# nirschl-lab/stain2stain

Measured on AMD Instinct MI355X. Metric: paired 256x256 stain tiles/sec (full CFM optimisation step), higher is better.
Workload: dtype bf16

## Files before the change

### include/stain2stain_hip.h

```cpp
#ifndef STAIN2STAIN_HIP_H
#define STAIN2STAIN_HIP_H

#ifdef __cplusplus
extern "C" {
#endif

#define S2S_OK 0
#define S2S_ERR_SHAPE (-1)
#define S2S_ERR_ALIGN (-2)
#define S2S_ERR_DTYPE (-3)
#define S2S_ERR_LAUNCH (-4)
#define S2S_ERR_NULL (-5)

#define S2S_BF16 0
#define S2S_F32 1

int s2s_conv3x3_stat_blocks(int dtype, int B, int H, int W, int Cout);
int s2s_conv3x3_nhwc(int dtype, const void* x0, int ld0, int c0, const void* x1, int ld1, int c1,
                     const void* w_packed, const float* bias, void* y, int ldy, float* stat_part,
                     const float* ep_scale, const float* ep_shift, int relu, int B, int H, int W, int Cout,
                     void* stream);

int s2s_conv3x3_ksplit(int dtype, int B, int H, int W, int Cout, int cin);
int s2s_conv3x3_nhwc_k(int dtype, const void* x0, int ld0, int c0, const void* x1, int ld1, int c1,
                       const void* w_packed, const float* bias, void* y, int ldy, float* stat_part,
                       const float* ep_scale, const float* ep_shift, int relu, float* kwork, int B, int H, int W,
                       int Cout, void* stream);
int s2s_conv3x3_stat_rows(int dtype, int B, int H, int W, int Cout, int c0, int c1, int ld0, int ld1, int has_bias);
int s2s_conv3x3_staged(int dtype, int B, int H, int W, int Cout, int c0, int c1, int ld0, int ld1, int ldy, int stats);
int s2s_conv3x3_family(int dtype, int B, int H, int W, int Cout, int c0, int c1, int ld0, int ld1, int ldy, int has_bias,
                       int has_affine, int stats, int stat_rows, int kwork);
int s2s_conv3x3_nhwc_s(int dtype, const void* x0, int ld0, int c0, const void* x1, int ld1, int c1, const void* w_packed,
                       const float* bias, void* y, int ldy, float* stat_part, int stat_rows, const float* ep_scale,
                       const float* ep_shift, int relu, float* kwork, int B, int H, int W, int Cout, void* stream);
int s2s_debug_conv_clock(long* out_host, int n);

int s2s_conv3x3_wgrad_splits(int dtype, int B, int H, int W, int Cin, int Cout);
int s2s_conv3x3_wgrad_nhwc(int dtype, const void* dy, int lddy, int Cout, const void* x0, int ld0, int c0,
                           const void* x1, int ld1, int c1, float* part, float* grad_oihw, int accumulate,
                           int B, int H, int W, void* stream);
int s2s_conv3x3_wgrad_phase(int dtype, const void* dy, int lddy, int Cout, const void* x0, int ld0, int c0,
                            const void* x1, int ld1, int c1, float* part, float* grad_oihw, int accumulate,
                            int B, int H, int W, int phases, void* stream);

int s2s_stem_stat_blocks(int B, int H, int W);
int s2s_stem_conv3x3_fwd(int dtype, const float* x_nchw, const float* w_oihw, const float* bias, void* y, int ldy,
                         float* stat_part, int B, int H, int W, int Cin, int Cout, void* stream);
int s2s_stem_wgrad_blocks(int B, int H, int W);
int s2s_stem_conv3x3_wgrad(int dtype, const void* dy, int lddy, const float* x_nchw, float* part, float* dw_oihw,
                           float* dbias, int accumulate, int B, int H, int W, int Cin, int Cout, void* stream);
int s2s_head_conv1x1_fwd(int dtype, const void* x, int ldx, const float* w, const float* bias, float* y_nchw, int B,
                         int H, int W, int C, int Cout, void* stream);
int s2s_head_wgrad_blocks(int B, int H, int W);
int s2s_head_conv1x1_bwd(int dtype, const float* dy_nchw, const void* x, int ldx, const float* w, void* dx, int lddx,
                         float* part, float* dw, float* dbias, int accumulate, int B, int H, int W, int C, int Cout,
                         void* stream);

int s2s_head_loss_blocks(int B, int H, int W);
int s2s_head_loss_fused(int dtype, const void* x, int ldx, const float* w, const float* bias, const float* u_nchw,
                        float* v_nchw, void* dx, int lddx, float grad_scale, float* part, double* lpart, float* dw,
                        float* dbias, float* loss, int accumulate, int B, int H, int W, int C, int Cout, void* stream);

int s2s_tail_blocks(int B, int H, int W);
int s2s_tail_fwd_loss(int dtype, const void* raw, int ldx, const float* scale, const float* shift, const float* mean,
                      const float* invstd, const float* w, const float* bias, const float* u_nchw, float* v_nchw,
                      float* g_nchw, float grad_scale, float* part, double* lpart, float* bnwork, float* dw,
                      float* dbias, float* loss, float* dgamma, float* dbeta, float* conv_dbias, int accumulate, int B,
                      int H, int W, int C, int Cout, void* stream);
int s2s_tail_bwd_apply(int dtype, const void* raw, int ldx, const float* g_nchw, const float* w, const float* scale,
                       const float* shift, const float* mean, const float* invstd, const float* gamma,
                       const float* bnwork, void* dx, int lddx, int B, int H, int W, int C, int Cout, void* stream);

int s2s_bn_finalize(const float* part, int nblk, int C, long count, const float* gamma, const float* beta,
                    float* running_mean, float* running_var, long* num_batches_tracked, float momentum, float eps,
                    float* mean, float* invstd, float* scale, float* shift, void* stream);
int s2s_bn_finalize_b(const float* part, int nblk, int C, long count, const float* gamma, const float* beta,
                      float* running_mean, float* running_var, long* num_batches_tracked, float momentum, float eps,
                      float* mean, float* invstd, float* scale, float* shift, const float* conv_bias, void* stream);
int s2s_bn_eval_prepare(int C, const float* gamma, const float* beta, const float* running_mean,
                        const float* running_var, float eps, float* scale, float* shift, void* stream);
int s2s_bn_relu_apply(int dtype, const void* x, int ldx, const float* scale, const float* shift, void* y, int ldy,
                      void* pool, int ldp, int B, int H, int W, int C, void* stream);
int s2s_maxpool2(int dtype, const void* x, int ldx, void* pool, int ldp, int B, int H, int W, int C, void* stream);
int s2s_bn_bwd_blocks(int B, int H, int W, int C);
int s2s_bn_relu_bwd(int dtype, const void* g1, int ldg1, const void* gp, int ldgp, const float* scale,
                    const float* shift, const void* x, int ldx, const float* mean, const float* invstd, const float* gamma, float* dgamma,
                    float* dbeta, float* dbias_conv, int accumulate, void* dx, int lddx, float* work, int B, int H,
                    int W, int C, void* stream);
int s2s_bn_partial_sums(const float* part, int nblk, int C, float* sums, void* stream);
int s2s_bn_relu_bwd_phase(int dtype, const void* g1, int ldg1, const void* gp, int ldgp, const float* scale,
                          const float* shift, const void* x, int ldx, const float* mean, const float* invstd,
                          const float* gamma, float* dgamma, float* dbeta, float* dbias_conv, int accumulate, void* dx,
                          int lddx, float* work, int B, int H, int W, int C, long count_total, int phases, void* stream);

int s2s_upsample2x_bilinear_ac_fwd(int dtype, const void* x, int ldx, const float* bias_nc, void* y, int ldy, int B,
                                   int Hin, int Win, int Hout, int Wout, int C, void* stream);
int s2s_upsample2x_bilinear_ac_bwd(int dtype, const void* dy, int lddy, void* dx, int lddx, int B, int Hin, int Win,
                                   int Hout, int Wout, int C, void* stream);
int s2s_pixel_sum(int dtype, const void* x, int ldx, float* out_nc, int B, int HW, int C, int accumulate,
                  void* stream);

int s2s_time_embedding(const float* t, float* out, int B, int dim, void* stream);
int s2s_linear_fwd(const float* x, const float* w, const float* bias, float* y, int B, int K, int N, void* stream);
int s2s_linear_bwd(const float* dy, const float* x, const float* w, float* dx, float* dw, float* db, int accumulate,
                   int B, int K, int N, void* stream);
int s2s_silu_fwd(const float* h, float* a, int n, void* stream);
int s2s_silu_bwd(const float* h, const float* da, float* dh, int n, void* stream);
int s2s_cfm_sample(const float* x0, const float* x1, const float* t, const float* eps, float sigma, float* xt,
                   float* ut, int B, long per_sample, void* stream);
int s2s_mse_loss(const float* v, const float* u, float* dv, float grad_scale, float* loss, double* work, long count,
                 void* stream);
int s2s_ode_error_norm(const float* e, const float* y0, const float* y1, float atol, float rtol, float* out,
                       double* work, long n, void* stream);
int s2s_axpy(float* x, const float* y, float a, long n, void* stream);
int s2s_dp_partials(long n);
int s2s_dp_init(int phase, const float* y, const float* k1, const float* fa, double* state, double* part, float* out,
                float* t_out, int* status, float atol, float rtol, int B, long n, void* stream);
int s2s_dp_stage(int i, const float* y, const float* k1, const float* k2, const float* k3, const float* k4,
                 const float* k5, const float* k6, const double* state, float* out, float* t_out, int B, long n,
                 void* stream);
int s2s_dp_error(const float* k1, const float* k2, const float* k3, const float* k4, const float* k5, const float* k6,
                 const float* k7, const float* y, const float* y_new, const double* state, double* part, float atol,
                 float rtol, int B, long n, void* stream);
int s2s_dp_control(double* state, const double* part, int* status, int max_steps, int B, long n, void* stream);
int s2s_dp_commit(float* y, const float* y_new, float* k1, const float* k7, const double* state, int B, long n,
                  void* stream);
int s2s_rk_stage(const float* x, const float* k1, const float* k2, const float* k3, float c1, float c2, float c3, int nk,
                 float* out, float* t_out, const float* table, const int* counter, int stages, int stage, int table_len,
                 int B, long n, void* stream);
int s2s_rk_combine(float* x, const float* k1, const float* k2, const float* k3, const float* k4, float c1, float c2,
                   float c3, float c4, int nk, int* counter, int B, long n, void* stream);
int s2s_fill_f32(float* x, float v, long n, void* stream);
int s2s_euler_tick(float* t, int n, const float* table, int* counter, void* stream);

int s2s_adam_step(float* p, const float* g, float* m, float* v, long n, int step, float lr, float beta1, float beta2,
                  float eps, float weight_decay, float grad_scale, void* stream);
int s2s_adam_step_dev(float* p, const float* g, float* m, float* v, long n, const float* hyper, void* stream);
long s2s_adam_multi_blocks(long n);
int s2s_adam_multi(const void* desc, int ntensors, long total, int step, float lr, float beta1, float beta2, float eps,
                   float weight_decay, float grad_scale, void* stream);
int s2s_adam_ema_step(float* p, const float* g, float* m, float* v, float* ema, long n, int step, float lr, float beta1,
                      float beta2, float eps, float weight_decay, float grad_scale, float ema_weight, void* stream);
int s2s_adam_ema_step_dev(float* p, const float* g, float* m, float* v, float* ema, long n, const float* hyper,
                          const float* ema_weight, void* stream);
long s2s_ema_multi_blocks(long n);
int s2s_ema_multi(const void* desc, int ntensors, long total, const float* weight, void* stream);
long s2s_pack_conv3x3_fwd_elems(int Cout, int Cin);
long s2s_pack_conv3x3_dgrad_elems(int Cout, int Cin);
int s2s_pack_conv3x3(int dtype, const float* w_oihw, void* w_fwd, void* w_dgrad, int Cout, int Cin, void* stream);
int s2s_pack_conv3x3_batched(int dtype, const void* desc, int nlayers, long total, void* stream);
int s2s_nchw_to_nhwc(int dtype, const float* x_nchw, void* y, int ldy, int B, int C, int H, int W, void* stream);
int s2s_nhwc_to_nchw(int dtype, const void* x, int ldx, float* y_nchw, int accumulate, int B, int C, int H, int W,
                     void* stream);

int s2s_paired_crop_flip_normalize(const void* src_u8, const void* tgt_u8, const int* params, float* out_src,
                                   float* out_tgt, int B, int Hs, int Ws, int S, void* stream);
int s2s_pil_resize_bilinear_normalize(const void* src_u8, void* tmp_u8, const int* bounds_h, const int* kk_h,
                                      int ksize_h, const int* bounds_v, const int* kk_v, int ksize_v, void* out_u8,
                                      float* out_f, int B, int Hs, int Ws, int Ho, int Wo, void* stream);

int s2s_region_gather(const void* img_u8, long pitch, int H, int W, int band_top, int band_h, const int* origins,
                      float* out, int B, int T, void* stream);
int s2s_region_blend(const float* tiles, int c0, const float* tiles1, int c1, const int* origins, int n, int T,
                     int overlap, float* acc, int band_rows, int H, int W, int r0, int r1, void* stream);
int s2s_region_finalize(float* acc, int band_rows, int W, int C, int r0, int r1, void* out_u8, long pitch_u8,
                        float* out_f, long pitch_f, int out_top, void* stream);

int s2s_region_tissue_count(const void* img_u8, long pitch, int H, int W, int band_top, int band_h, const int* origins,
                            int n, int T, int white, int black, int* counts, void* stream);
int s2s_region_skip_weight(const int* origins, int n, int T, int overlap, float* ws, int band_rows, int H, int W,
                           int r0, int r1, void* stream);
int s2s_region_finalize_mixed(float* acc, float* ws, int band_rows, int W, int C, int r0, int r1, const void* src_u8,
                              long src_pitch, int src_top, void* out_u8, long pitch_u8, float* out_f, long pitch_f,
                              int out_top, void* stream);

int s2s_seg_loss(const float* z, const float* g, float* dz, float* out, double* work, long n, float smooth,
                 float dice_weight, float grad_scale, void* stream);
int s2s_seg_loss_multiclass(const float* z, const long* target, float* dz, float* out, double* work, long B, long HW,
                            int C, int ignore_index, float smooth, float dice_weight, float grad_scale, void* stream);

int s2s_seg_eval_binary(const float* z, const float* g, float* out, long* counts, double* work, long n, float smooth,
                        float dice_weight, void* stream);
int s2s_seg_eval_multiclass(const float* z, const long* target, float* out, long* counts, double* work, long B,
                            long HW, int C, int ignore_index, float smooth, float dice_weight, void* stream);
int s2s_head_mse_eval_blocks(int B, int H, int W, int C);
int s2s_head_mse_eval(int dtype, const void* x, int ldx, const float* w, const float* bias, const float* u_nchw,
                      float* loss, double* lpart, int B, int H, int W, int C, int Cout, void* stream);

int s2s_image_quality_blocks(int H, int W, int win);
int s2s_image_quality_f32(const float* a, const float* b, int B, int C, int H, int W, int quantize, int win,
                          const float* taps, float k1, float k2, double* part, void* stream);
int s2s_image_quality_u8(const void* a, long pitch_a, long img_a, const void* b, long pitch_b, long img_b, int B,
                         int band_top, int band_h, int H, int W, int by0, int nby, int win, const float* taps, float k1,
                         float k2, double* part, void* stream);
int s2s_image_quality_finalize(const double* part, int B, int C, int H, int W, int win, float range, float* out,
                               void* stream);

int s2s_stain_quant_chunks(int cell_h, int cell_w);
int s2s_stain_quant_u8(const void* a, long pitch_a, long img_a, const void* b, long pitch_b, long img_b, int paired,
                       int B, int band_top, int band_h, int H, int W, int cell_h, int cell_w, int g0, int ng,
                       const float* od_table, const float* unmix, int white, int black, int stain, double* part,
                       void* stream);
int s2s_stain_quant_f32(const float* a, const float* b, int paired, int B, int H, int W, const float* od_table,
                        const float* unmix, int white, int black, int stain, double* part, void* stream);
int s2s_stain_quant_finalize(const double* part, long owners, int nchunk, int paired, long* counts, double* sums,
                             float* out, void* stream);
int s2s_stain_separate(const void* img, int is_f32, long pitch, long img_stride, int B, int H, int W,
                       const float* od_table, const float* unmix, float* out, void* stream);

long s2s_stain_moments_slots(int B, int H, int W);
int s2s_stain_moments_u8(const void* img, long pitch, long img_stride, int B, int band_top, int band_h, int H, int W,
                         const int* q_table, int u_beta, int black, long* part, void* stream);
int s2s_stain_moments_finalize(const long* part, long nslots, long* out, void* stream);
int s2s_stain_angle_hist_u8(const void* img, long pitch, long img_stride, int B, int band_top, int band_h, int H, int W,
                            const float* od_table, const float* plane, int u_beta, int black, int reset, long* hist,
                            void* stream);
int s2s_stain_conc_hist_u8(const void* img, long pitch, long img_stride, int B, int band_top, int band_h, int H, int W,
                           const float* od_table, const float* unmix, int u_beta, int black, int reset, long* hist,
                           void* stream);
int s2s_stain_normalize_u8(const void* img, long pitch, long img_stride, int B, int H, int W, const float* od_table,
                           const float* coef, void* out, long out_pitch, long out_img, int out_f32, void* stream);

int s2s_weighted_mse(const float* v, const float* u, const float* mask, float* dv, float* out, double* work, long B,
                     int C, long HW, float roi_lambda, float grad_scale, void* stream);
int s2s_charbonnier_roi(const float* pred, const float* truth, const float* mask, float* out, double* work, long B,
                        int C, long HW, float eps_charb, float eps_area, void* stream);
int s2s_class_embed_add(const float* temb, const float* table, const long* y, float* out, int B, int dim,
                        void* stream);
int s2s_class_embed_bwd(const float* dout, const long* y, float* dtable, int accumulate, int B, int dim,
                        int num_classes, void* stream);

int s2s_instnorm_blocks(int B, int H, int W, int C);
int s2s_instnorm_lrelu_fwd(int dtype, const void* x, int ldx, const float* gamma, const float* beta, void* y, int ldy,
                           float* work, float* stats, int B, int H, int W, int C, float eps, float slope,
                           void* stream);
int s2s_instnorm_lrelu_bwd(int dtype, const void* g, int ldg, const void* x, int ldx, const float* stats, void* dx,
                           int lddx, float* dgamma, float* dbeta, int accumulate, float* work, int B, int H, int W,
                           int C, float slope, void* stream);

int s2s_conv2x2_stat_blocks(int B, int H, int W, int Cout);
int s2s_conv2x2_nhwc(int dtype, const void* x, int ldx, int cin, const void* w_packed, const float* bias, void* y,
                     int ldy, float* stat_part, int B, int H, int W, int Cout, int pad, void* stream);
int s2s_space_to_depth_pad1(int dtype, const void* x, int ldx, void* xs, int ldxs, int inverse, int B, int H, int W,
                            int C, void* stream);
int s2s_channel_sum_blocks(long npix, int C);
int s2s_channel_sum(int dtype, const void* x, int ldx, float* work, float* out, long npix, int C, int accumulate,
                    void* stream);
int s2s_pack_conv4x4(const float* w_oihw, void* wf, void* wd, int Cout, int Cin, int stride, void* stream);
int s2s_conv4x4s1_nhwc(int dtype, const void* x, int ldx, int cin, const void* w_packed, const float* bias, void* y,
                       int ldy, float* stat_part, int B, int H, int W, int Cout, int pad, void* stream);
int s2s_conv4x4s1_wgrad_splits(int B, int H, int W, int Cin, int Cout);
// ... 72 lines not shown
```

### stain2stain_amd/csrc/resample.hip

```cpp
#include "common.h"
#include <stdlib.h>

namespace {

struct Axis {
  int i0, i1;
  float w0, w1;
};

__device__ __forceinline__ Axis ac_axis(int dst, int n_in, float scale) {
  Axis a;
  const float src = scale * (float)dst;
  a.i0 = (int)src;
  if (a.i0 > n_in - 1) a.i0 = n_in - 1;
  a.i1 = a.i0 + (a.i0 < n_in - 1 ? 1 : 0);
  a.w1 = src - (float)a.i0;
  a.w0 = 1.f - a.w1;
  return a;
}

__device__ __forceinline__ int rs_pcb(int C) {
  int p = 1;
  while (p < 32 && p * 8 < C) p <<= 1;
  return p;
// ... 13 lines not shown
  const int nrows = B * Hout;
  for (int row0 = blockIdx.x * band; row0 < nrows; row0 += gridDim.x * band)
  for (int row = row0; row < row0 + band && row < nrows; ++row) {
    const int n = row / Hout, oy = row - n * Hout;
    const int uy = oy - padT;
    const bool row_in = uy >= 0 && uy < Hu;
    const Axis ay = ac_axis(row_in ? uy : 0, Hin, sh);
    const T* const r0 = x + ((long)n * Hin + ay.i0) * Win * ldx;
    const T* const r1 = x + ((long)n * Hin + ay.i1) * Win * ldx;
    T* const yr = y + (long)row * Wout * ldy;
    for (int pb = 0; pb < cp; pb += PCB) {
      const int c8 = (pb + pc) * 8;
      if (pb + pc >= cp) continue;
      float bv[8];
#pragma unroll
      for (int k = 0; k < 8; ++k) bv[k] = BIAS ? bias[(long)n * C + c8 + k] : 0.f;
      for (int ox = slot; ox < Wout; ox += WL) {
        const int ux = ox - padL;
        f32x8 o;
        if (!row_in || ux < 0 || ux >= Wu) {
#pragma unroll
          for (int k = 0; k < 8; ++k) o.v[k] = 0.f;
        } else {
          const Axis ax = ac_axis(ux, Win, sw);
          const int o0 = ax.i0 * ldx + c8, o1 = ax.i1 * ldx + c8;
          const f32x8 v00 = load8(r0 + o0), v01 = load8(r0 + o1), v10 = load8(r1 + o0), v11 = load8(r1 + o1);
#pragma unroll
          for (int k = 0; k < 8; ++k) {
            const float b = bv[k];
            o.v[k] = ay.w0 * (ax.w0 * (v00.v[k] + b) + ax.w1 * (v01.v[k] + b)) +
                     ay.w1 * (ax.w0 * (v10.v[k] + b) + ax.w1 * (v11.v[k] + b));
          }
        }
        store8(yr + ox * ldy + c8, o);
      }
    }
  }
}

template <typename T>
__global__ void upsample2x_bwd_kernel(const T* __restrict__ dy, int lddy, T* __restrict__ dx, int lddx, int B,
                                      int Hin, int Win, int Hout, int Wout, int padT, int padL, int C) {
  const int cp = C >> 3;
  const int Hu = 2 * Hin, Wu = 2 * Win;
  const float sh = Hu > 1 ? (float)(Hin - 1) / (float)(Hu - 1) : 0.f;
  const float sw = Wu > 1 ? (float)(Win - 1) / (float)(Wu - 1) : 0.f;
  const int total = B * Hin * Win * cp;
  for (int i = blockIdx.x * blockDim.x + threadIdx.x; i < total; i += gridDim.x * blockDim.x) {
    const int t0 = i / cp, c8 = (i - t0 * cp) * 8;
    const int t1 = t0 / Win, ix = t0 - t1 * Win;
    const int n = t1 / Hin, iy = t1 - n * Hin;
    int y_lo, y_hi, x_lo, x_hi;
    if (Hin == 1) { y_lo = 0; y_hi = Hu - 1; }
    else {
      y_lo = (int)floorf((float)(iy - 1) / sh) - 1; y_hi = (int)ceilf((float)(iy + 1) / sh) + 1;
      if (y_lo < 0) y_lo = 0;
      if (y_hi > Hu - 1) y_hi = Hu - 1;
    }
    if (Win == 1) { x_lo = 0; x_hi = Wu - 1; }
    else {
      x_lo = (int)floorf((float)(ix - 1) / sw) - 1; x_hi = (int)ceilf((float)(ix + 1) / sw) + 1;
      if (x_lo < 0) x_lo = 0;
      if (x_hi > Wu - 1) x_hi = Wu - 1;
    }
    constexpr int NSLOT = 12;
    float wxs[NSLOT];
#pragma unroll
    for (int j = 0; j < NSLOT; ++j) {
      const int ux = x_lo + j;
      float wx = 0.f;
      if (ux <= x_hi) {
        const Axis ax = ac_axis(ux, Win, sw);
        if (ax.i0 == ix) wx += ax.w0;
        if (ax.i1 == ix) wx += ax.w1;
        const int ox = ux + padL;
        if (ox < 0 || ox >= Wout) wx = 0.f;
      }
      wxs[j] = wx;
    }
    f32x8 acc;
#pragma unroll
    for (int k = 0; k < 8; ++k) acc.v[k] = 0.f;
    for (int uy = y_lo; uy <= y_hi; ++uy) {
      const Axis ay = ac_axis(uy, Hin, sh);
      float wy = 0.f;
      if (ay.i0 == iy) wy += ay.w0;
      if (ay.i1 == iy) wy += ay.w1;
      const int oy = uy + padT;
      if (wy == 0.f || oy < 0 || oy >= Hout) continue;
      const T* const rowp = dy + (((long)n * Hout + oy) * Wout + x_lo + padL) * lddy + c8;
#pragma unroll
      for (int j = 0; j < NSLOT; ++j) {
        if (wxs[j] == 0.f) continue;
        const f32x8 g = load8(rowp + (long)j * lddy);
        const float w = wy * wxs[j];
#pragma unroll
        for (int k = 0; k < 8; ++k) acc.v[k] += w * g.v[k];
      }
    }
    store8(dx + (((long)n * Hin + iy) * Win + ix) * lddx + c8, acc);
  }
}

__device__ __forceinline__ float ac_weight_of(int dst, int n_in, float scale, int src_index) {
  const Axis a = ac_axis(dst, n_in, scale);
  return (a.i0 == src_index ? a.w0 : 0.f) + (a.i1 == src_index ? a.w1 : 0.f);
}

template <typename T>
__global__ void upsample2x_bwd_win_kernel(const T* __restrict__ dy, int lddy, T* __restrict__ dx, int lddx, int B,
                                          int Hin, int Win, int Hout, int Wout, int padT, int padL, int C) {
  const int cp = C >> 3;
  const int Hu = 2 * Hin, Wu = 2 * Win;
  const float sh = (float)(Hin - 1) / (float)(Hu - 1), sw = (float)(Win - 1) / (float)(Wu - 1);
  const int total = B * Hin * Win * cp;
  for (int i = blockIdx.x * blockDim.x + threadIdx.x; i < total; i += gridDim.x * blockDim.x) {
    const int t0 = i / cp, c8 = (i - t0 * cp) * 8;
    const int t1 = t0 / Win, ix = t0 - t1 * Win;
    const int n = t1 / Hin, iy = t1 - n * Hin;
    int uy0 = (int)floorf((float)(iy - 1) / sh) - 1, ux0 = (int)floorf((float)(ix - 1) / sw) - 1;
    if (uy0 < 0) uy0 = 0;
    if (ux0 < 0) ux0 = 0;
    for (int t = 0; t < 8 && uy0 < Hu - 1 && ac_weight_of(uy0, Hin, sh, iy) == 0.f; ++t) ++uy0;
    for (int t = 0; t < 8 && ux0 < Wu - 1 && ac_weight_of(ux0, Win, sw, ix) == 0.f; ++t) ++ux0;
    float wy[5], wx[5];
    int oyc[5], oxc[5];
#pragma unroll
    for (int j = 0; j < 5; ++j) {
      const int uy = uy0 + j, ux = ux0 + j;
      const int oy = uy + padT, ox = ux + padL;
      wy[j] = (uy <= Hu - 1 && oy >= 0 && oy < Hout) ? ac_weight_of(uy, Hin, sh, iy) : 0.f;
      wx[j] = (ux <= Wu - 1 && ox >= 0 && ox < Wout) ? ac_weight_of(ux, Win, sw, ix) : 0.f;
      oyc[j] = oy < 0 ? 0 : (oy > Hout - 1 ? Hout - 1 : oy);
      oxc[j] = ox < 0 ? 0 : (ox > Wout - 1 ? Wout - 1 : ox);
    }
    f32x8 acc;
#pragma unroll
    for (int k = 0; k < 8; ++k) acc.v[k] = 0.f;
#pragma unroll
    for (int j = 0; j < 5; ++j) {
      const T* const rowp = dy + ((long)n * Hout + oyc[j]) * Wout * lddy + c8;
#pragma unroll
      for (int m = 0; m < 5; ++m) {
        const f32x8 g = load8(rowp + (long)oxc[m] * lddy);
        const float w = wy[j] * wx[m];
#pragma unroll
        for (int k = 0; k < 8; ++k) acc.v[k] = fmaf(w, g.v[k], acc.v[k]);
      }
    }
    store8(dx + (((long)n * Hin + iy) * Win + ix) * lddx + c8, acc);
  }
}

template <typename T>
__global__ void pixel_sum_kernel(const T* __restrict__ x, int ldx, float* __restrict__ out, int HW, int C,
                                 int accumulate) {
  const int n = blockIdx.y;
  const int c = blockIdx.x * 64 + (threadIdx.x & 63);
  const int rg = threadIdx.x >> 6;
  float s = 0.f;
  if (c < C)
    for (int p = rg; p < HW; p += 4) s += to_f32(x[((long)n * HW + p) * ldx + c]);
  __shared__ float red[4][64];
  red[rg][threadIdx.x & 63] = s;
  __syncthreads();
  if (rg == 0 && c < C) {
    s = red[0][threadIdx.x] + red[1][threadIdx.x] + red[2][threadIdx.x] + red[3][threadIdx.x];
    out[(long)n * C + c] = accumulate ? out[(long)n * C + c] + s : s;
  }
}

inline int ew_grid(long total) {
  long b = (total + 255) / 256;
  if (b > 8192) b = 8192;
  if (b < 1) b = 1;
  return (int)b;
}

}

extern "C" int s2s_upsample2x_bilinear_ac_fwd(int dtype, const void* x, int ldx, const float* bias_nc, void* y,
                                              int ldy, int B, int Hin, int Win, int Hout, int Wout, int C,
                                              void* stream) {
  if (!x || !y) return S2S_ERR_NULL;
  if (B <= 0 || Hin <= 0 || Win <= 0 || C <= 0 || (C % 8) || (ldx % 8) || (ldy % 8)) return S2S_ERR_SHAPE;
  if (Hout < 2 * Hin || Wout < 2 * Win) return S2S_ERR_SHAPE;
  const int padT = (Hout - 2 * Hin) / 2, padL = (Wout - 2 * Win) / 2;
  if ((long)Win * ldx >= (1L << 31) || (long)Wout * ldy >= (1L << 31) || (long)B * Hout >= (1L << 31))
    return S2S_ERR_SHAPE;
  hipStream_t s = (hipStream_t)stream;
  const long rows = (long)B * Hout;
  static const int band_env = [] { const char* e = getenv("S2S_UP_BAND"); return e ? atoi(e) : 0; }();
  const int band = band_env > 0 ? band_env : (rows >= 4096 ? 4 : rows >= 2048 ? 2 : 1);
  const long nwg = (rows + band - 1) / band;
  const dim3 grid((unsigned)(nwg < 65535 * 4 ? nwg : 65535 * 4));
#define S2S_UP(TT, BB)                                                                                          \
  hipLaunchKernelGGL((upsample2x_fwd_kernel<TT, BB>), grid, dim3(256), 0, s, (const TT*)x, ldx, bias_nc, (TT*)y, \
                     ldy, B, Hin, Win, Hout, Wout, padT, padL, C, band)
  if (dtype == S2S_BF16) { if (bias_nc) S2S_UP(bf16_t, true); else S2S_UP(bf16_t, false); }
  else if (dtype == S2S_F32) { if (bias_nc) S2S_UP(float, true); else S2S_UP(float, false); }
  else return S2S_ERR_DTYPE;
#undef S2S_UP
  S2S_LAUNCH_CHECK();
  return S2S_OK;
}

extern "C" int s2s_upsample2x_bilinear_ac_bwd(int dtype, const void* dy, int lddy, void* dx, int lddx, int B, int Hin,
                                              int Win, int Hout, int Wout, int C, void* stream) {
  if (!dy || !dx) return S2S_ERR_NULL;
  if (B <= 0 || Hin <= 0 || Win <= 0 || C <= 0 || (C % 8) || (lddy % 8) || (lddx % 8)) return S2S_ERR_SHAPE;
  if (Hout < 2 * Hin || Wout < 2 * Win) return S2S_ERR_SHAPE;
  const int padT = (Hout - 2 * Hin) / 2, padL = (Wout - 2 * Win) / 2;
  const long total = (long)B * Hin * Win * (C / 8);
  if (total >= (1L << 31) - (1L << 22)) return S2S_ERR_SHAPE;
  hipStream_t s = (hipStream_t)stream;
  const dim3 grid(ew_grid(total));
  const bool win = Hin > 3 && Win > 3;
  if (dtype != S2S_BF16 && dtype != S2S_F32) return S2S_ERR_DTYPE;
#define S2S_UPB(KERN, TT)                                                                                            \
  hipLaunchKernelGGL(KERN<TT>, grid, dim3(256), 0, s, (const TT*)dy, lddy, (TT*)dx, lddx, B, Hin, Win, Hout, Wout,   \
                     padT, padL, C)
  if (dtype == S2S_BF16) { if (win) S2S_UPB(upsample2x_bwd_win_kernel, bf16_t); else S2S_UPB(upsample2x_bwd_kernel, bf16_t); }
  else { if (win) S2S_UPB(upsample2x_bwd_win_kernel, float); else S2S_UPB(upsample2x_bwd_kernel, float); }
#undef S2S_UPB
  S2S_LAUNCH_CHECK();
  return S2S_OK;
}

extern "C" int s2s_pixel_sum(int dtype, const void* x, int ldx, float* out_nc, int B, int HW, int C, int accumulate,
                             void* stream) {
  if (!x || !out_nc) return S2S_ERR_NULL;
  if (B <= 0 || HW <= 0 || C <= 0) return S2S_ERR_SHAPE;
  hipStream_t s = (hipStream_t)stream;
  dim3 grid(cdiv(C, 64), B);
  if (dtype == S2S_BF16)
    hipLaunchKernelGGL(pixel_sum_kernel<bf16_t>, grid, dim3(256), 0, s, (const bf16_t*)x, ldx, out_nc, HW, C, accumulate);
  else if (dtype == S2S_F32)
    hipLaunchKernelGGL(pixel_sum_kernel<float>, grid, dim3(256), 0, s, (const float*)x, ldx, out_nc, HW, C, accumulate);
  else return S2S_ERR_DTYPE;
  S2S_LAUNCH_CHECK();
  return S2S_OK;
}
```

### stain2stain_amd/ops.py

```python
from __future__ import annotations

import contextlib
import ctypes
import os
import sys
from typing import Optional, Tuple

import torch

from . import _native

BF16, F32 = 0, 1


def _dt(t: torch.Tensor) -> int:
    if t.dtype == torch.bfloat16:
        return BF16
    if t.dtype == torch.float32:
        return F32
    raise RuntimeError(f"stain2stain_amd: unsupported activation dtype {t.dtype}")


_raw_stream = getattr(torch._C, "_cuda_getCurrentRawStream", None)
_raw_device = getattr(torch._C, "_cuda_getDevice", None)
# ... 370 lines not shown


def tail_fusable(C: int, cout: int) -> bool:
    pcb = C // 8
    return C % 8 == 0 and 1 <= pcb <= 64 and pcb & (pcb - 1) == 0 and 1 <= cout <= 4


@_timed("tail_fwd_loss")
def tail_fwd_loss(raw: torch.Tensor, stats: torch.Tensor, w: torch.Tensor, bias: Optional[torch.Tensor],
                  u_nchw: torch.Tensor, dw: torch.Tensor, dbias: Optional[torch.Tensor], dgamma: torch.Tensor,
                  dbeta: torch.Tensor, dbias_conv: Optional[torch.Tensor], want_v: bool = False,
                  grad_scale: float = 1.0, accumulate: bool = False):
    B, H, W, C = raw.shape
    cout = w.shape[0]
    if not tail_fusable(C, cout):
        raise RuntimeError(f"stain2stain_amd: the fused tail does not take C = {C}, cout = {cout}")
    px, ldx = _nhwc(raw)
    dev = raw.device
    g = torch.empty((B, cout, H, W), dtype=torch.float32, device=dev)
    v = torch.empty((B, cout, H, W), dtype=torch.float32, device=dev) if want_v else None
    nb = _L().s2s_tail_blocks(B, H, W)
    part = torch.empty((nb, cout, C + 1), dtype=torch.float32, device=dev)
    lpart = torch.empty((nb,), dtype=torch.float64, device=dev)
    work = torch.empty((2 * C * _L().s2s_bn_bwd_blocks(B, H, W, C) + 2 * C,), dtype=torch.float32, device=dev)
    loss = torch.empty((), dtype=torch.float32, device=dev)
    rc = _L().s2s_tail_fwd_loss(_dt(raw), px, ldx, stats[2].data_ptr(), stats[3].data_ptr(), stats[0].data_ptr(),
                                stats[1].data_ptr(), _f32(w.reshape(cout, C)), _f32(bias), _f32(u_nchw), _f32(v),
                                _f32(g), float(grad_scale), _f32(part), lpart.data_ptr(), _f32(work),
                                _f32(dw.reshape(cout, C)), _f32(dbias), loss.data_ptr(), _f32(dgamma), _f32(dbeta),
                                _f32(dbias_conv), int(accumulate), B, H, W, C, cout, _stream())
    _native.check(rc, "tail_fwd_loss")
    return loss, g, v, work


@_timed("tail_bwd_apply")
def tail_bwd_apply(raw: torch.Tensor, stats: torch.Tensor, w: torch.Tensor, g: torch.Tensor, gamma: torch.Tensor,
                   work: torch.Tensor) -> torch.Tensor:
    B, H, W, C = raw.shape
    cout = w.shape[0]
    px, ldx = _nhwc(raw)
    if tuple(g.shape) != (B, cout, H, W) or work.numel() != 2 * C * _L().s2s_bn_bwd_blocks(B, H, W, C) + 2 * C:
        raise RuntimeError("stain2stain_amd: tail_bwd_apply operands do not belong to this tail_fwd_loss")
    dx = torch.empty((B, H, W, C), dtype=raw.dtype, device=raw.device)
    rc = _L().s2s_tail_bwd_apply(_dt(raw), px, ldx, _f32(g), _f32(w.reshape(cout, C)), stats[2].data_ptr(),
                                 stats[3].data_ptr(), stats[0].data_ptr(), stats[1].data_ptr(), _f32(gamma),
                                 _f32(work), dx.data_ptr(), C, B, H, W, C, cout, _stream())
    _native.check(rc, "tail_bwd_apply")
    return dx


@_timed("bn_finalize")
def bn_finalize(stat: torch.Tensor, count: int, gamma, beta, running_mean, running_var, num_batches,
                momentum: float = 0.1, eps: float = 1e-5, conv_bias: Optional[torch.Tensor] = None):
    _, C, nblk = stat.shape
    dev = stat.device
    out = torch.empty((4, C), dtype=torch.float32, device=dev)
    rc = _L().s2s_bn_finalize_b(_f32(stat), nblk, C, count, _f32(gamma), _f32(beta), _f32(running_mean),
                                _f32(running_var), 0 if num_batches is None else num_batches.data_ptr(), momentum, eps,
                                out[0].data_ptr(), out[1].data_ptr(), out[2].data_ptr(), out[3].data_ptr(),
                                _f32(conv_bias), _stream())
    _native.check(rc, "bn_finalize")
    return out


def bn_partial_sums(stat: torch.Tensor) -> torch.Tensor:
    _, C, nblk = stat.shape
    sums = torch.empty((2, C), dtype=torch.float32, device=stat.device)
    _native.check(_L().s2s_bn_partial_sums(_f32(stat), nblk, C, _f32(sums), _stream()), "bn_partial_sums")
    return sums


def bn_eval_prepare(gamma, beta, rmean, rvar, eps: float = 1e-5):
    C = gamma.numel()
    out = torch.empty((2, C), dtype=torch.float32, device=gamma.device)
    rc = _L().s2s_bn_eval_prepare(C, _f32(gamma), _f32(beta), _f32(rmean), _f32(rvar), eps, out[0].data_ptr(),
                                  out[1].data_ptr(), _stream())
    _native.check(rc, "bn_eval_prepare")
    return out


@_timed("bn_relu_apply")
def bn_relu_apply(x: torch.Tensor, scale: torch.Tensor, shift: torch.Tensor, out: Optional[torch.Tensor] = None,
                  pool: Optional[torch.Tensor] = None, want_pool: bool = False):
    B, H, W, C = x.shape
    px, ldx = _nhwc(x)
    if out is None:
        out = torch.empty((B, H, W, C), dtype=x.dtype, device=x.device)
    py, ldy = _nhwc(out)
    pp, ldp = 0, 8
    if want_pool and pool is None:
        pool = torch.empty((B, H // 2, W // 2, C), dtype=x.dtype, device=x.device)
    if pool is not None:
        pp, ldp = _nhwc(pool)
    rc = _L().s2s_bn_relu_apply(_dt(x), px, ldx, _f32(scale), _f32(shift), py, ldy, pp, ldp, B, H, W, C, _stream())
    _native.check(rc, "bn_relu_apply")
    return out, pool


@_timed("maxpool2")
def maxpool2(x: torch.Tensor) -> torch.Tensor:
    B, H, W, C = x.shape
    px, ldx = _nhwc(x)
    pool = torch.empty((B, H // 2, W // 2, C), dtype=x.dtype, device=x.device)
    rc = _L().s2s_maxpool2(_dt(x), px, ldx, pool.data_ptr(), C, B, H, W, C, _stream())
    _native.check(rc, "maxpool2")
    return pool


@_timed("bn_relu_bwd")
def bn_relu_bwd(g1: Optional[torch.Tensor], gp: Optional[torch.Tensor], x: torch.Tensor,
                stats: torch.Tensor, gamma: torch.Tensor, dgamma: torch.Tensor, dbeta: torch.Tensor,
                dbias_conv: Optional[torch.Tensor], accumulate: bool = False, exchange=None,
                count_total: Optional[int] = None) -> torch.Tensor:
    B, H, W, C = x.shape
    px, ldx = _nhwc(x)
    p1, ld1 = (0, 8) if g1 is None else _nhwc(g1)
    p2, ld2 = (0, 8) if gp is None else _nhwc(gp)
    dx = torch.empty((B, H, W, C), dtype=x.dtype, device=x.device)
    nb = _L().s2s_bn_bwd_blocks(B, H, W, C)
    work = torch.empty((4 * nb * C + 2 * C,), dtype=torch.float32, device=x.device)
    if exchange is not None:
        for phase in (1, 2):
            rc = _L().s2s_bn_relu_bwd_phase(_dt(x), p1, ld1, p2, ld2, stats[2].data_ptr(), stats[3].data_ptr(), px, ldx,
                                            stats[0].data_ptr(), stats[1].data_ptr(),
                                            _f32(gamma), _f32(dgamma), _f32(dbeta), _f32(dbias_conv), int(accumulate),
                                            dx.data_ptr(), C, _f32(work), B, H, W, C,
                                            int(count_total if count_total is not None else B * H * W), phase, _stream())
            _native.check(rc, "bn_relu_bwd")
            if phase == 1:
                exchange(work[4 * nb * C:])
        return dx
    rc = _L().s2s_bn_relu_bwd(_dt(x), p1, ld1, p2, ld2, stats[2].data_ptr(), stats[3].data_ptr(), px, ldx,
                              stats[0].data_ptr(), stats[1].data_ptr(),
                              _f32(gamma), _f32(dgamma), _f32(dbeta), _f32(dbias_conv), int(accumulate),
                              dx.data_ptr(), C, _f32(work), B, H, W, C, _stream())
    _native.check(rc, "bn_relu_bwd")
    return dx


@_timed("upsample2x_fwd")
def upsample2x_fwd(x: torch.Tensor, out: torch.Tensor, bias_nc: Optional[torch.Tensor] = None) -> None:
    B, Hin, Win, C = x.shape
    _, Hout, Wout, Co = out.shape
    if Co != C or out.dtype != x.dtype:
        raise RuntimeError("stain2stain_amd: upsample output slice mismatch")
    px, ldx = _nhwc(x)
    py, ldy = _nhwc(out)
    rc = _L().s2s_upsample2x_bilinear_ac_fwd(_dt(x), px, ldx, _f32(bias_nc), py, ldy, B, Hin, Win, Hout, Wout, C,
                                             _stream())
    _native.check(rc, "upsample2x_fwd")


@_timed("upsample2x_bwd")
def upsample2x_bwd(dy: torch.Tensor, hin: int, win: int) -> torch.Tensor:
    B, Hout, Wout, C = dy.shape
    pdy, lddy = _nhwc(dy)
    dx = torch.empty((B, hin, win, C), dtype=dy.dtype, device=dy.device)
    rc = _L().s2s_upsample2x_bilinear_ac_bwd(_dt(dy), pdy, lddy, dx.data_ptr(), C, B, hin, win, Hout, Wout, C,
                                             _stream())
    _native.check(rc, "upsample2x_bwd")
    return dx


def pixel_sum(x: torch.Tensor) -> torch.Tensor:
    B, H, W, C = x.shape
    px, ldx = _nhwc(x)
    out = torch.empty((B, C), dtype=torch.float32, device=x.device)
    rc = _L().s2s_pixel_sum(_dt(x), px, ldx, _f32(out), B, H * W, C, 0, _stream())
    _native.check(rc, "pixel_sum")
    return out


def time_embedding(t: torch.Tensor, dim: int) -> torch.Tensor:
    t = t.reshape(-1).to(torch.float32).contiguous()
    out = torch.empty((t.numel(), dim), dtype=torch.float32, device=t.device)
    _native.check(_L().s2s_time_embedding(_f32(t), _f32(out), t.numel(), dim, _stream()), "time_embedding")
    return out


def linear_fwd(x: torch.Tensor, w: torch.Tensor, b: Optional[torch.Tensor]) -> torch.Tensor:
    B, K = x.shape
    N = w.shape[0]
    y = torch.empty((B, N), dtype=torch.float32, device=x.device)
    _native.check(_L().s2s_linear_fwd(_f32(x), _f32(w), _f32(b), _f32(y), B, K, N, _stream()), "linear_fwd")
    return y


def linear_bwd(dy: torch.Tensor, x: torch.Tensor, w: torch.Tensor, dw: torch.Tensor, db: Optional[torch.Tensor],
               need_dx: bool = True, accumulate: bool = False) -> Optional[torch.Tensor]:
    B, K = x.shape
    N = w.shape[0]
    dx = torch.empty((B, K), dtype=torch.float32, device=x.device) if need_dx else None
    _native.check(_L().s2s_linear_bwd(_f32(dy), _f32(x), _f32(w), _f32(dx), _f32(dw), _f32(db), int(accumulate), B, K,
                                      N, _stream()), "linear_bwd")
    return dx


def silu_fwd(h: torch.Tensor) -> torch.Tensor:
    a = torch.empty_like(h)
    _native.check(_L().s2s_silu_fwd(_f32(h), _f32(a), h.numel(), _stream()), "silu_fwd")
    return a


def silu_bwd(h: torch.Tensor, da: torch.Tensor) -> torch.Tensor:
    dh = torch.empty_like(h)
    _native.check(_L().s2s_silu_bwd(_f32(h), _f32(da), _f32(dh), h.numel(), _stream()), "silu_bwd")
    return dh


@_timed("cfm_sample")
def cfm_sample(x0: torch.Tensor, x1: torch.Tensor, t: torch.Tensor, sigma: float = 0.0,
               eps: Optional[torch.Tensor] = None):
    xt = torch.empty_like(x0)
    ut = torch.empty_like(x0)
    B = x0.shape[0]
    _native.check(_L().s2s_cfm_sample(_f32(x0), _f32(x1), _f32(t), _f32(eps), float(sigma), _f32(xt), _f32(ut), B,
                                      x0.numel() // B, _stream()), "cfm_sample")
    return xt, ut


@_timed("mse_loss")
def mse_loss(v: torch.Tensor, u: torch.Tensor, want_grad: bool = True, grad_scale: float = 1.0):
    loss = torch.empty((), dtype=torch.float32, device=v.device)
    dv = torch.empty_like(v) if want_grad else None
    work = torch.empty((1024,), dtype=torch.float64, device=v.device)
    _native.check(_L().s2s_mse_loss(_f32(v), _f32(u), _f32(dv), float(grad_scale), loss.data_ptr(), work.data_ptr(),
                                    v.numel(), _stream()), "mse_loss")
    return loss, dv


def seg_loss(z: torch.Tensor, g: torch.Tensor, smooth: float = 1.0, dice_weight: float = 0.5, want_grad: bool = True,
             grad_scale: float = 1.0):
    z = z.contiguous()
    g = g.to(torch.float32).contiguous()
    out = torch.empty((3,), dtype=torch.float32, device=z.device)
    dz = torch.empty_like(z) if want_grad else None
    work = torch.empty((512 * 4 + 4,), dtype=torch.float64, device=z.device)
    _native.check(_L().s2s_seg_loss(_f32(z), _f32(g), _f32(dz), _f32(out), work.data_ptr(), z.numel(), float(smooth),
                                    float(dice_weight), float(grad_scale), _stream()), "seg_loss")
    return out, dz


def seg_loss_multiclass(z: torch.Tensor, target: torch.Tensor, ignore_index: int = -100, smooth: float = 1.0,
                        dice_weight: float = 0.5, want_grad: bool = True, grad_scale: float = 1.0,
                        validate: bool = True):
    if z.dim() != 4 or target.dim() != 3 or target.shape != (z.shape[0], z.shape[2], z.shape[3]):
        raise RuntimeError("stain2stain_amd: seg_loss_multiclass wants logits [B,C,H,W] and target [B,H,W]")
    B, C, H, W = z.shape
    z = z.contiguous()
    target = target.to(torch.int64).contiguous()
    if validate:
        lo, hi = int(target.min()), int(target.max())
        if lo < 0 or hi >= C:
            raise RuntimeError(f"stain2stain_amd: class index out of range [0, {C}) in segmentation target "
                               f"(min {lo}, max {hi})")
    out = torch.empty((3,), dtype=torch.float32, device=z.device)
    dz = torch.empty_like(z) if want_grad else None
    work = torch.empty((513 * 26,), dtype=torch.float64, device=z.device)
    _native.check(_L().s2s_seg_loss_multiclass(_f32(z), target.data_ptr(), _f32(dz), _f32(out), work.data_ptr(), B,
                                               H * W, C, int(ignore_index), float(smooth), float(dice_weight),
                                               float(grad_scale), _stream()), "seg_loss_multiclass")
    return out, dz


EV_BLOCKS = 512


def _gpu_f32_operand(t: torch.Tensor, what: str) -> torch.Tensor:
    if not t.is_cuda:
        raise RuntimeError(f"stain2stain_amd: {what} is not on the GPU (there is no CPU path)")
    if t.dtype != torch.float32:
        raise RuntimeError(f"stain2stain_amd: {what} must be float32, got {t.dtype}")
    return t.contiguous()


def _binary_mask(g: torch.Tensor) -> torch.Tensor:
    if g.dtype in (torch.bool, torch.uint8):
        return g.to(torch.float32).contiguous()
    if g.dtype != torch.float32:
        raise RuntimeError(f"stain2stain_amd: mask must be float32 (0/1), uint8 or bool, got {g.dtype}")
    return g.contiguous()


@_timed("seg_eval_binary")
def seg_eval_binary(z: torch.Tensor, g: torch.Tensor, smooth: float = 1.0, dice_weight: float = 0.5):
    if z.dim() != 4 or z.shape[1] != 1:
        raise RuntimeError(f"stain2stain_amd: seg_eval_binary wants logits [B,1,H,W], got {tuple(z.shape)}")
    if g.dim() == 3:
        g = g.unsqueeze(1)
    if tuple(g.shape) != tuple(z.shape):
        raise RuntimeError(f"stain2stain_amd: mask shape {tuple(g.shape)} does not match logits {tuple(z.shape)}")
    if g.device != z.device:
        raise RuntimeError("stain2stain_amd: logits and mask are on different devices")
    z, g = _gpu_f32_operand(z, "logits"), _binary_mask(g)
    out = torch.empty((5,), dtype=torch.float32, device=z.device)
    counts = torch.empty((4,), dtype=torch.int64, device=z.device)
    work = _workspace(z.device, 2 * EV_BLOCKS * 8, "seg_eval").view(torch.float64)
    _native.check(_L().s2s_seg_eval_binary(_f32(z), _f32(g), _f32(out), counts.data_ptr(), work.data_ptr(), z.numel(),
                                           float(smooth), float(dice_weight), _stream()), "seg_eval_binary")
    return out, counts


@_timed("seg_eval_multiclass")
def seg_eval_multiclass(z: torch.Tensor, target: torch.Tensor, ignore_index: int = -100, smooth: float = 1.0,
                        dice_weight: float = 0.5):
    if z.dim() != 4:
        raise RuntimeError(f"stain2stain_amd: seg_eval_multiclass wants logits [B,C,H,W], got {tuple(z.shape)}")
    B, C, H, W = z.shape
    if not 2 <= C <= 8:
        raise RuntimeError(f"stain2stain_amd: seg_eval_multiclass supports 2 <= C <= 8 classes, got {C}")
    if target.dim() == 4 and target.shape[1] == 1:
        target = target[:, 0]
    if tuple(target.shape) != (B, H, W):
        raise RuntimeError(f"stain2stain_amd: target shape {tuple(target.shape)} does not match logits {tuple(z.shape)}")
# ... 1093 lines not shown
```

Before: 2300.

## Add 2x2-quad upsample backward kernel and unroll pixel_sum loads

Adds a new bilinear upsample backward kernel in which each thread computes a 2x2 quad of input pixels from a shared 6x6 window of output gradients. Neighbouring outputs reuse the same loads instead of each pixel gathering its own 5x5 window. The kernel also uses an XCD-aware workgroup remap and sched barriers. Separately, pixel_sum is unrolled by 16 so more loads are in flight. A reference path and a family-query entry point are kept for testing, at the cost of extra code and higher register pressure.

```diff
diff --git a/include/stain2stain_hip.h b/include/stain2stain_hip.h
--- a/include/stain2stain_hip.h
+++ b/include/stain2stain_hip.h
@@ -97,6 +97,9 @@
                                    int Hin, int Win, int Hout, int Wout, int C, void* stream);
 int s2s_upsample2x_bilinear_ac_bwd(int dtype, const void* dy, int lddy, void* dx, int lddx, int B, int Hin, int Win,
                                    int Hout, int Wout, int C, void* stream);
+int s2s_upsample2x_bilinear_ac_bwd_ref(int dtype, const void* dy, int lddy, void* dx, int lddx, int B, int Hin,
+                                       int Win, int Hout, int Wout, int C, void* stream);
+int s2s_upsample2x_bwd_family(int lddy, int lddx, int B, int Hin, int Win, int Hout, int Wout, int C, int reference);
 int s2s_pixel_sum(int dtype, const void* x, int ldx, float* out_nc, int B, int HW, int C, int accumulate,
                   void* stream);
 
diff --git a/stain2stain_amd/csrc/resample.hip b/stain2stain_amd/csrc/resample.hip
--- a/stain2stain_amd/csrc/resample.hip
+++ b/stain2stain_amd/csrc/resample.hip
@@ -189,6 +189,137 @@
   }
 }
 
+template <typename T> struct Raw8;
+template <> struct Raw8<bf16_t> { bf16x8 a; };
+template <> struct Raw8<float> { f32x4 a, b; };
+__device__ __forceinline__ Raw8<bf16_t> load_raw8(const bf16_t* p) {
+  Raw8<bf16_t> r;
+  r.a = *reinterpret_cast<const bf16x8*>(p);
+  return r;
+}
+__device__ __forceinline__ Raw8<float> load_raw8(const float* p) {
+  Raw8<float> r;
+  r.a = *reinterpret_cast<const f32x4*>(p);
+  r.b = *reinterpret_cast<const f32x4*>(p + 4);
+  return r;
+}
+__device__ __forceinline__ f32x8 widen8(const Raw8<bf16_t>& r) {
+  f32x8 o;
+#pragma unroll
+  for (int i = 0; i < 8; ++i) o.v[i] = (float)r.a[i];
+  return o;
+}
+__device__ __forceinline__ f32x8 widen8(const Raw8<float>& r) {
+  f32x8 o;
+#pragma unroll
+  for (int i = 0; i < 4; ++i) { o.v[i] = r.a[i]; o.v[4 + i] = r.b[i]; }
+  return o;
+}
+
+__device__ __forceinline__ void pin8(f32x8& r) {
+#pragma unroll
+  for (int i = 0; i < 8; ++i) asm volatile("" : "+v"(r.v[i]));
+}
+
+template <typename T>
+__global__ __launch_bounds__(256, sizeof(T) == 2 ? 4 : 2) void upsample2x_bwd_quad_kernel(const T* __restrict__ dy, int lddy,
+                                                                  T* __restrict__ dx, int lddx, int B, int Hin,
+                                                                  int Win, int Hout, int Wout, int padT, int padL,
+                                                                  int C, int nwork) {
+  const int cp = C >> 3;
+  const int Hu = 2 * Hin, Wu = 2 * Win;
+  const float sh = (float)(Hin - 1) / (float)(Hu - 1), sw = (float)(Win - 1) / (float)(Wu - 1);
+  const int PCB = rs_pcb(C), WL = 256 / PCB;
+  const int pc = threadIdx.x & (PCB - 1), slot = threadIdx.x / PCB;
+  const int HP = (Hin + 1) >> 1, WP = (Win + 1) >> 1;
+  const int nwg = gridDim.x, q = nwg >> 3, r = nwg & 7, cls = blockIdx.x & 7;
+  const int wgid = (cls < r ? cls * (q + 1) : r * (q + 1) + (cls - r) * q) + (blockIdx.x >> 3);
+  const int chunk = wgid / nwork, work = wgid - chunk * nwork;
+  const int n = work / HP, iy0 = min(2 * (work - n * HP), Hin - 2);
+  const int piece = chunk * PCB + pc;
+  if (piece >= cp) return;
+  const int c8 = piece * 8;
+
+  float wyA[4], wyB[4];
+  const T* rowp[6];
+#pragma unroll
+  for (int j = 0; j < 6; ++j) {
+    const int uy = 2 * iy0 - 1 + j;
+    const bool in = uy >= 0 && uy <= Hu - 1;
+    if (j < 4) wyA[j] = in ? ac_weight_of(uy, Hin, sh, iy0) : 0.f;
+    if (j >= 2) wyB[j - 2] = in ? ac_weight_of(uy, Hin, sh, iy0 + 1) : 0.f;
+    int oy = uy + padT;
+    oy = oy < 0 ? 0 : (oy > Hout - 1 ? Hout - 1 : oy);
+    rowp[j] = dy + ((long)n * Hout + oy) * Wout * lddy;
+  }
+  T* const dr0 = dx + ((long)n * Hin + iy0) * Win * lddx + c8;
+  T* const dr1 = dr0 + (long)Win * lddx;
+
+#pragma unroll 1
+  for (int px = slot; px < WP; px += WL) {
+    const int ix0 = min(2 * px, Win - 2);
+    float wxA[4], wxB[4];
+    int off[6];
+#pragma unroll
+    for (int m = 0; m < 6; ++m) {
+      const int ux = 2 * ix0 - 1 + m;
+      const bool in = ux >= 0 && ux <= Wu - 1;
+      if (m < 4) wxA[m] = in ? ac_weight_of(ux, Win, sw, ix0) : 0.f;
+      if (m >= 2) wxB[m - 2] = in ? ac_weight_of(ux, Win, sw, ix0 + 1) : 0.f;
+      int ox = ux + padL;
+      ox = ox < 0 ? 0 : (ox > Wout - 1 ? Wout - 1 : ox);
+      off[m] = ox * lddy + c8;
+    }
+    f32x8 a00, a01, a10, a11;
+#pragma unroll
+    for (int k = 0; k < 8; ++k) a00.v[k] = a01.v[k] = a10.v[k] = a11.v[k] = 0.f;
+#pragma unroll
+    for (int j = 0; j < 6; ++j) {
+      Raw8<T> cur[6];
+#pragma unroll
+      for (int m = 0; m < 6; ++m) cur[m] = load_raw8(rowp[j] + off[m]);
+      f32x8 g[6];
+#pragma unroll
+      for (int m = 0; m < 6; ++m) g[m] = widen8(cur[m]);
+      if (j < 4) {
+#pragma unroll
+        for (int m = 0; m < 4; ++m) {
+          const float w = wyA[j] * wxA[m];
+#pragma unroll
+          for (int k = 0; k < 8; ++k) a00.v[k] = fmaf(w, g[m].v[k], a00.v[k]);
+        }
+#pragma unroll
+        for (int m = 0; m < 4; ++m) {
+          const float w = wyA[j] * wxB[m];
+#pragma unroll
+          for (int k = 0; k < 8; ++k) a01.v[k] = fmaf(w, g[m + 2].v[k], a01.v[k]);
+        }
+      }
+      if (j >= 2) {
+#pragma unroll
+        for (int m = 0; m < 4; ++m) {
+          const float w = wyB[j - 2] * wxA[m];
+#pragma unroll
+          for (int k = 0; k < 8; ++k) a10.v[k] = fmaf(w, g[m].v[k], a10.v[k]);
+        }
+#pragma unroll
+        for (int m = 0; m < 4; ++m) {
+          const float w = wyB[j - 2] * wxB[m];
+#pragma unroll
+          for (int k = 0; k < 8; ++k) a11.v[k] = fmaf(w, g[m + 2].v[k], a11.v[k]);
+        }
+      }
+      if (j < 4) { pin8(a00); pin8(a01); }
+      if (j >= 2) { pin8(a10); pin8(a11); }
+      __builtin_amdgcn_sched_barrier(0);
+    }
+    store8(dr0 + ix0 * lddx, a00);
+    store8(dr0 + (ix0 + 1) * lddx, a01);
+    store8(dr1 + ix0 * lddx, a10);
+    store8(dr1 + (ix0 + 1) * lddx, a11);
+  }
+}
+
 template <typename T>
 __global__ void pixel_sum_kernel(const T* __restrict__ x, int ldx, float* __restrict__ out, int HW, int C,
                                  int accumulate) {
@@ -196,8 +327,19 @@
   const int c = blockIdx.x * 64 + (threadIdx.x & 63);
   const int rg = threadIdx.x >> 6;
   float s = 0.f;
-  if (c < C)
-    for (int p = rg; p < HW; p += 4) s += to_f32(x[((long)n * HW + p) * ldx + c]);
+  if (c < C) {
+    constexpr int U = 16;
+    const T* const xp = x + (long)n * HW * ldx + c;
+    int p = rg;
+    for (; p + 4 * (U - 1) < HW; p += 4 * U) {
+      float v[U];
+#pragma unroll
+      for (int u = 0; u < U; ++u) v[u] = to_f32(xp[(long)(p + 4 * u) * ldx]);
+#pragma unroll
+      for (int u = 0; u < U; ++u) s += v[u];
+    }
+    for (; p < HW; p += 4) s += to_f32(xp[(long)p * ldx]);
+  }
   __shared__ float red[4][64];
   red[rg][threadIdx.x & 63] = s;
   __syncthreads();
@@ -242,8 +384,20 @@
   return S2S_OK;
 }
 
-extern "C" int s2s_upsample2x_bilinear_ac_bwd(int dtype, const void* dy, int lddy, void* dx, int lddx, int B, int Hin,
-                                              int Win, int Hout, int Wout, int C, void* stream) {
+namespace {
+
+enum UpBwdFamily { kUpBwdGather = 0, kUpBwdWindow = 1, kUpBwdQuad = 2 };
+
+int upsample2x_bwd_family(int lddy, int lddx, int B, int Hin, int Win, int Wout, int C, bool reference) {
+  if (!(Hin > 3 && Win > 3)) return kUpBwdGather;
+  const long nwork = (long)B * ((Hin + 1) / 2);
+  const bool quad = !reference && Hin <= 4096 && Win <= 4096 && (long)Wout * lddy < (1L << 31) &&
+                    (long)Win * lddx < (1L << 31) && nwork * cdiv(C / 8, 32) < (1L << 31);
+  return quad ? kUpBwdQuad : kUpBwdWindow;
+}
+
+int upsample2x_bwd_launch(int dtype, const void* dy, int lddy, void* dx, int lddx, int B, int Hin, int Win, int Hout,
+                          int Wout, int C, void* stream, bool reference) {
   if (!dy || !dx) return S2S_ERR_NULL;
   if (B <= 0 || Hin <= 0 || Win <= 0 || C <= 0 || (C % 8) || (lddy % 8) || (lddx % 8)) return S2S_ERR_SHAPE;
   if (Hout < 2 * Hin || Wout < 2 * Win) return S2S_ERR_SHAPE;
@@ -252,9 +406,23 @@
   if (total >= (1L << 31) - (1L << 22)) return S2S_ERR_SHAPE;
   hipStream_t s = (hipStream_t)stream;
   const dim3 grid(ew_grid(total));
-  const bool win = Hin > 3 && Win > 3;
   if (dtype != S2S_BF16 && dtype != S2S_F32) return S2S_ERR_DTYPE;
-#define S2S_UPB(KERN, TT)                                                                                            \
+  const int family = upsample2x_bwd_family(lddy, lddx, B, Hin, Win, Wout, C, reference);
+  const bool win = family != kUpBwdGather;
+  const int nchunk = cdiv(C / 8, 32);
+  const long nwork = (long)B * ((Hin + 1) / 2);
+  if (family == kUpBwdQuad) {
+    const dim3 qgrid((unsigned)(nwork * nchunk));
+    if (dtype == S2S_BF16)
+      hipLaunchKernelGGL(upsample2x_bwd_quad_kernel<bf16_t>, qgrid, dim3(256), 0, s, (const bf16_t*)dy, lddy,
+                         (bf16_t*)dx, lddx, B, Hin, Win, Hout, Wout, padT, padL, C, (int)nwork);
+    else
+      hipLaunchKernelGGL(upsample2x_bwd_quad_kernel<float>, qgrid, dim3(256), 0, s, (const float*)dy, lddy, (float*)dx,
+                         lddx, B, Hin, Win, Hout, Wout, padT, padL, C, (int)nwork);
+    S2S_LAUNCH_CHECK();
+    return S2S_OK;
+  }
+#define S2S_UPB(KERN, TT)                                                                                           \
   hipLaunchKernelGGL(KERN<TT>, grid, dim3(256), 0, s, (const TT*)dy, lddy, (TT*)dx, lddx, B, Hin, Win, Hout, Wout,   \
                      padT, padL, C)
   if (dtype == S2S_BF16) { if (win) S2S_UPB(upsample2x_bwd_win_kernel, bf16_t); else S2S_UPB(upsample2x_bwd_kernel, bf16_t); }
@@ -262,6 +430,26 @@
 #undef S2S_UPB
   S2S_LAUNCH_CHECK();
   return S2S_OK;
+}
+
+}
+
+extern "C" int s2s_upsample2x_bilinear_ac_bwd(int dtype, const void* dy, int lddy, void* dx, int lddx, int B, int Hin,
+                                              int Win, int Hout, int Wout, int C, void* stream) {
+  return upsample2x_bwd_launch(dtype, dy, lddy, dx, lddx, B, Hin, Win, Hout, Wout, C, stream, false);
+}
+
+extern "C" int s2s_upsample2x_bilinear_ac_bwd_ref(int dtype, const void* dy, int lddy, void* dx, int lddx, int B,
+                                                  int Hin, int Win, int Hout, int Wout, int C, void* stream) {
+  return upsample2x_bwd_launch(dtype, dy, lddy, dx, lddx, B, Hin, Win, Hout, Wout, C, stream, true);
+}
+
+extern "C" int s2s_upsample2x_bwd_family(int lddy, int lddx, int B, int Hin, int Win, int Hout, int Wout, int C,
+                                         int reference) {
+  if (B <= 0 || Hin <= 0 || Win <= 0 || C <= 0 || (C % 8) || (lddy % 8) || (lddx % 8)) return S2S_ERR_SHAPE;
+  if (Hout < 2 * Hin || Wout < 2 * Win) return S2S_ERR_SHAPE;
+  if ((long)B * Hin * Win * (C / 8) >= (1L << 31) - (1L << 22)) return S2S_ERR_SHAPE;
+  return upsample2x_bwd_family(lddy, lddx, B, Hin, Win, Wout, C, reference != 0);
 }
 
 extern "C" int s2s_pixel_sum(int dtype, const void* x, int ldx, float* out_nc, int B, int HW, int C, int accumulate,
diff --git a/stain2stain_amd/ops.py b/stain2stain_amd/ops.py
--- a/stain2stain_amd/ops.py
+++ b/stain2stain_amd/ops.py
@@ -546,14 +546,22 @@
 
 
 @_timed("upsample2x_bwd")
-def upsample2x_bwd(dy: torch.Tensor, hin: int, win: int) -> torch.Tensor:
+def upsample2x_bwd(dy: torch.Tensor, hin: int, win: int, _reference: bool = False) -> torch.Tensor:
     B, Hout, Wout, C = dy.shape
     pdy, lddy = _nhwc(dy)
     dx = torch.empty((B, hin, win, C), dtype=dy.dtype, device=dy.device)
-    rc = _L().s2s_upsample2x_bilinear_ac_bwd(_dt(dy), pdy, lddy, dx.data_ptr(), C, B, hin, win, Hout, Wout, C,
-                                             _stream())
+    fn = _L().s2s_upsample2x_bilinear_ac_bwd_ref if _reference else _L().s2s_upsample2x_bilinear_ac_bwd
+    rc = fn(_dt(dy), pdy, lddy, dx.data_ptr(), C, B, hin, win, Hout, Wout, C, _stream())
     _native.check(rc, "upsample2x_bwd")
     return dx
+
+
+def upsample2x_bwd_family(dy: torch.Tensor, hin: int, win: int, _reference: bool = False) -> int:
+    B, Hout, Wout, C = dy.shape
+    rc = _L().s2s_upsample2x_bwd_family(dy.stride(2), C, B, hin, win, Hout, Wout, C, int(_reference))
+    if rc < 0:
+        _native.check(rc, "upsample2x_bwd_family")
+    return rc
 
 
 def pixel_sum(x: torch.Tensor) -> torch.Tensor:
```

New measurement: 2333 (median of 6 runs). 1.01x the previous value.
